# khajash/gym_puzzles

Hardware: AMD Instinct MI355X
Metric: env-steps/sec (whole node) at N envs/GPU (higher is better)
Workload: dtype f32 (engine) + f64 (env arithmetic)

## Files before the change

### gym_puzzles_amd/build.py

```python
from __future__ import annotations

import os
import re
import subprocess
import sys
from concurrent.futures import ThreadPoolExecutor

HERE = os.path.dirname(os.path.abspath(__file__))
CSRC = os.path.join(HERE, "csrc")
OUT = os.path.join(HERE, "libmrp.so")
with open(os.path.join(CSRC, "mrp_config.h")) as _f:
    N_ENVS = len(re.findall(r"^\s*X\(\d+,", _f.read(), re.M))
SOURCES = ([(f, f + ".o", None) for f in ("mrp_kernels.hip", "mrp_tables.cpp", "mrp_norm.hip")]
           + [("mrp_unit.hip", f"mrp_env{e}.o", e) for e in range(N_ENVS)])
HEADERS = ("mrp_math.h", "mrp_config.h", "mrp_world.h", "mrp_env.h", "mrp_tables.h", "mrp_ops.h", "mrp_lane.h", "mrp_render.h")


def deps(csrc: str = CSRC) -> list[str]:
    return [os.path.join(csrc, f) for f in sorted({s for s, _, _ in SOURCES}) + list(HEADERS)] + [
        os.path.join(HERE, "..", "include", "mrp.h"), os.path.abspath(__file__)]


_MAX_ILP = ["-mllvm", "-amdgpu-sched-strategy=max-ilp"]
_ILP_LOOPS = ["-DMRP_SOLVE_NOINLINE_LANES"] + _MAX_ILP
_LANES_PAIRS = ["-DMRP_LANES_PAIRS=1"]
_GRANULES = ["-DMRP_CONTACT_GRANULES=1"]
_ITER_ILP = ["-mllvm", "-amdgpu-sched-strategy=iterative-ilp"]
_BFREE = ["-DMRP_VEL_BFREE=1", "-DMRP_VEL_PICK2=1", "-DMRP_VEL_VTCROSS=1"]
_FRESH = ["-DMRP_FRESH_REGS=1"]
_BFREE_LANES = ["-DMRP_VEL_BFREE=1", "-DMRP_VEL_BFREE_LANES=1"]
_W4 = ["-DMRP_STEP_WAVES_PER_EU=4"]
UNIT_FLAGS = {0: _LANES_PAIRS + _ITER_ILP + _FRESH + _BFREE_LANES + _W4, 1: _MAX_ILP,
              2: _GRANULES + _MAX_ILP + _BFREE, 4: _ILP_LOOPS + _BFREE,
              5: _LANES_PAIRS + _ITER_ILP + _FRESH + _BFREE_LANES + _W4}
FLAGS = ["--offload-arch=gfx950", "-O3", "-std=c++17", "-ffp-contract=off", "-fno-fast-math",
         "-fno-gpu-flush-denormals-to-zero", "-fhip-fp32-correctly-rounded-divide-sqrt", "-fno-strict-aliasing",
         "-fno-slp-vectorize", "-fPIC", "-Wno-pass-failed"]


def hipcc() -> str:
    for c in (os.environ.get("HIPCC"), "/opt/rocm/bin/hipcc", "hipcc"):
        if c and (os.path.exists(c) or c == "hipcc"):
            return c
    return "hipcc"


def up_to_date() -> bool:
    if not os.path.exists(OUT):
        return False
    t = os.path.getmtime(OUT)
    return all(os.path.getmtime(d) <= t for d in deps() if os.path.exists(d))


def build(force: bool = False, verbose: bool = False, out: str = OUT, defines=(), jobs: int | None = None,
          only_envs=None, csrc: str = CSRC) -> str:
    if not force and out == OUT and up_to_date():
        return out
    objdir = os.path.join(HERE, "build", os.path.basename(out) + ".obj")
    os.makedirs(objdir, exist_ok=True)
    dflags = [f"-D{d}" for d in defines]
    srcs = [os.path.join(csrc, s) for s, _, _ in SOURCES]
    objs = [os.path.join(objdir, o) for _, o, _ in SOURCES]
    todo = list(range(len(SOURCES)))
    dep_files = deps(csrc)
    if only_envs is not None:
        assert out != OUT, "only_envs builds a variant library, never the default one"
        base = os.path.join(HERE, "build", os.path.basename(OUT) + ".obj")
        todo = [i for i, (_, _, e) in enumerate(SOURCES) if e is None or e in only_envs]
        newest_dep = max(os.path.getmtime(d) for d in dep_files if os.path.exists(d) and d.endswith((".h", ".hip", ".cpp")))
        for i, (_, o, _) in enumerate(SOURCES):
            if i not in todo:
                objs[i] = os.path.join(base, o)
                if not os.path.exists(objs[i]):
                    raise FileNotFoundError(f"{objs[i]}: build the default library first")
                if os.path.getmtime(objs[i]) < newest_dep and not os.environ.get("MRP_ALLOW_STALE_UNITS"):
                    raise RuntimeError(f"{objs[i]} is older than a source or header it depends on: rebuild the default "
                                       "library (python -m gym_puzzles_amd.build) before a variant")

    extra = os.environ.get("MRP_EXTRA_FLAGS", "").split() if out != OUT else []

    headers = [d for d in dep_files if d.endswith(".h")]
    newest_header = max(os.path.getmtime(d) for d in headers if os.path.exists(d))

    def compile_one(i: int) -> None:
        env = SOURCES[i][2]
        unit = [] if env is None else (UNIT_FLAGS.get(env, []) if not extra else []) + [f"-DMRP_ENV={env}"]
        cmd = [hipcc()] + FLAGS + unit + extra + dflags + ["-c", srcs[i], "-o", objs[i]]
        stamp = objs[i] + ".cmd"
        line = " ".join(cmd)
        if not force and os.path.exists(objs[i]) and os.path.exists(stamp):
            t = os.path.getmtime(objs[i])
            with open(stamp) as f:
                same = f.read() == line
            if same and t >= os.path.getmtime(srcs[i]) and t >= newest_header:
                return
        if verbose:
            print(line, flush=True)
        subprocess.run(cmd, check=True)
        with open(stamp, "w") as f:
            f.write(line)

    jobs = jobs or max(1, min(len(SOURCES), os.cpu_count() or 1, int(os.environ.get("MAX_JOBS", "16"))))
    order = sorted(todo, key=lambda i: SOURCES[i][2] is None)
    with ThreadPoolExecutor(jobs) as ex:
        list(ex.map(compile_one, order))
    cmd = [hipcc()] + FLAGS + ["-shared"] + objs + ["-o", out + ".tmp"]
    if verbose:
        print(" ".join(cmd), flush=True)
    subprocess.run(cmd, check=True)
    os.replace(out + ".tmp", out)
    return out


if __name__ == "__main__":
    if "--stamps" in sys.argv:
        print(build(verbose=True, out=os.path.join(HERE, "libmrp_stamps.so"), defines=("MRP_STAMPS",)))
    elif "--progress" in sys.argv:
        print(build(verbose=True, out=os.path.join(HERE, "libmrp_progress.so"), defines=("MRP_PROGRESS",)))
    elif "--variant" in sys.argv:
        i = sys.argv.index("--variant")
        args = sys.argv[i + 2:]
        envs = [int(a) for a in args if not a.startswith("-D")]
        defs = [a[2:] for a in args if a.startswith("-D")]
        print(build(verbose=True, out=os.path.abspath(sys.argv[i + 1]), defines=defs, only_envs=envs))
    else:
        print(build(force="--force" in sys.argv, verbose=True))
```

### gym_puzzles_amd/csrc/mrp_math.h

```cpp
#pragma once
#include <hip/hip_runtime.h>
#include <stdint.h>

#define MRP_HD __host__ __device__ __forceinline__

namespace mrp {

struct V2 { float x, y; };
struct Rot { float s, c; };
struct Xf { V2 p; Rot q; };

MRP_HD V2 v2(float x, float y) { V2 r; r.x = x; r.y = y; return r; }
MRP_HD V2 vadd(V2 a, V2 b) { return v2(a.x + b.x, a.y + b.y); }
MRP_HD V2 vsub(V2 a, V2 b) { return v2(a.x - b.x, a.y - b.y); }
MRP_HD V2 vmul(float s, V2 a) { return v2(s * a.x, s * a.y); }
MRP_HD V2 vneg(V2 a) { return v2(-a.x, -a.y); }
MRP_HD float vdot(V2 a, V2 b) { return a.x * b.x + a.y * b.y; }
MRP_HD float vcross(V2 a, V2 b) { return a.x * b.y - a.y * b.x; }
MRP_HD V2 vcross_vs(V2 a, float s) { return v2(s * a.y, -s * a.x); }
MRP_HD V2 vcross_sv(float s, V2 a) { return v2(-s * a.y, s * a.x); }
MRP_HD float vlensq(V2 a) { return a.x * a.x + a.y * a.y; }
MRP_HD float vlen(V2 a) { return sqrtf(a.x * a.x + a.y * a.y); }
MRP_HD float vnormalize(V2& a) {
    float length = sqrtf(a.x * a.x + a.y * a.y);
// ... 34 lines not shown
constexpr double SC_HPI_INV = 0x1.45F306DC9C883p+23, SC_HPI = 0x1.921FB54442D18p0;
constexpr double SC_C0 = 0x1p0, SC_C1 = -0x1.ffffffd0c621cp-2, SC_C2 = 0x1.55553e1068f19p-5,
                 SC_C3 = -0x1.6c087e89a359dp-10, SC_C4 = 0x1.99343027bf8c3p-16;
constexpr double SC_S1 = -0x1.555545995a603p-3, SC_S2 = 0x1.1107605230bc4p-7, SC_S3 = -0x1.994eb3774cf24p-13;

MRP_HD double sc_sign(int n) { return ((n + 1) & 2) ? -1.0 : 1.0; }

MRP_HD uint32_t f2u(float f) { union { float f; uint32_t u; } x; x.f = f; return x.u; }
MRP_HD float u2f(uint32_t u) { union { float f; uint32_t u; } x; x.u = u; return x.f; }
MRP_HD uint32_t abstop12(float x) { return (f2u(x) >> 20) & 0x7ff; }

MRP_HD float sincos_poly(double x, double x2, bool neg, int n) {
    if ((n & 1) == 0) {
        double x3 = x * x2;
        double s1 = fma(x2, SC_S3, SC_S2);
        double x7 = x3 * x2;
        double s = fma(x3, SC_S1, x);
        return (float)fma(x7, s1, s);
    } else {
        double x4 = x2 * x2;
        double c2 = fma(x2, SC_C4, SC_C3);
        double c1 = fma(x2, SC_C1, SC_C0);
        double x6 = x4 * x2;
        double c = fma(x4, SC_C2, c1);
        float r = (float)fma(x6, c2, c);
        return neg ? -r : r;
    }
}

MRP_HD double reduce_fast(double x, int* np) {
    double r = x * SC_HPI_INV;
    int n = ((int32_t)r + 0x800000) >> 24;
    *np = n;
    return fma(-(double)n, SC_HPI, x);
}

MRP_HD double reduce_large(uint32_t xi, int* np) {
    const uint32_t inv_pio4[24] = {0xa2, 0xa2f9, 0xa2f983, 0xa2f9836e, 0xf9836e4e, 0x836e4e44, 0x6e4e4415, 0x4e441529,
        0x441529fc, 0x1529fc27, 0x29fc2757, 0xfc2757d1, 0x2757d1f5, 0x57d1f534, 0xd1f534dd, 0xf534ddc0,
        0x34ddc0db, 0xddc0db62, 0xc0db6295, 0xdb629599, 0x6295993c, 0x95993c43, 0x993c4390, 0x3c439041};
    const uint32_t* arr = &inv_pio4[(xi >> 26) & 15];
    int shift = (xi >> 23) & 7;
    uint64_t n, res0, res1, res2;
    xi = (xi & 0xffffff) | 0x800000;
    xi <<= shift;
    res0 = xi * arr[0];
    res1 = (uint64_t)xi * arr[4];
    res2 = (uint64_t)xi * arr[8];
    res0 = (res2 >> 32) | (res0 << 32);
    res0 += res1;
    n = (res0 + (1ULL << 61)) >> 62;
    res0 -= n << 62;
    double x = (double)(int64_t)res0;
    *np = (int)n;
    return x * 0x1.921FB54442D18p-62;
}

MRP_HD float g_sinf(float y) {
    double x = y, s; int n;
    if (abstop12(y) < abstop12(0x1.921FB6p-1f)) {
        s = x * x;
        if (abstop12(y) < abstop12(0x1p-12f)) return y;
        return sincos_poly(x, s, false, 0);
    } else if (abstop12(y) < abstop12(120.0f)) {
        x = reduce_fast(x, &n);
        s = sc_sign(n);
        return sincos_poly(x * s, x * x, (n & 2) != 0, n);
    } else if (abstop12(y) < abstop12(__builtin_inff())) {
        uint32_t xi = f2u(y); int sign = xi >> 31;
        x = reduce_large(xi, &n);
        s = sc_sign(n + sign);
        return sincos_poly(x * s, x * x, ((n + sign) & 2) != 0, n);
    }
    return (y - y) / (y - y);
}

MRP_HD float g_cosf(float y) {
    double x = y, s; int n;
    if (abstop12(y) < abstop12(0x1.921FB6p-1f)) {
        double x2 = x * x;
        if (abstop12(y) < abstop12(0x1p-12f)) return 1.0f;
        return sincos_poly(x, x2, false, 1);
    } else if (abstop12(y) < abstop12(120.0f)) {
        x = reduce_fast(x, &n);
        s = sc_sign(n);
        return sincos_poly(x * s, x * x, (n & 2) != 0, n ^ 1);
    } else if (abstop12(y) < abstop12(__builtin_inff())) {
        uint32_t xi = f2u(y); int sign = xi >> 31;
        x = reduce_large(xi, &n);
        s = sc_sign(n + sign);
        return sincos_poly(x * s, x * x, ((n + sign) & 2) != 0, n ^ 1);
    }
    return (y - y) / (y - y);
}

MRP_HD Rot rot_fast(float y) {
    const double x = y;
    const double r = x * SC_HPI_INV;
    const int n = ((int32_t)r + 0x800000) >> 24;
    const double xr = fma(-(double)n, SC_HPI, x);
    const double xs = ((n + 1) & 2) ? -xr : xr;
    const double x2 = xr * xr;
    const double x3 = xs * x2;
    const double s1 = fma(x2, SC_S3, SC_S2);
    const double x7 = x3 * x2;
    const double ss = fma(x3, SC_S1, xs);
    const float ps = (float)fma(x7, s1, ss);
    const double x4 = x2 * x2;
    const double c2 = fma(x2, SC_C4, SC_C3);
    const double c1 = fma(x2, SC_C1, SC_C0);
    const double x6 = x4 * x2;
    const double cc = fma(x4, SC_C2, c1);
    const float pc0 = (float)fma(x6, c2, cc);
    const float pc = (n & 2) ? -pc0 : pc0;
    const bool odd = (n & 1) != 0;
    const bool tiny = abstop12(y) < abstop12(0x1p-12f);
    Rot q;
    q.s = tiny ? y : (odd ? pc : ps);
    q.c = tiny ? 1.0f : (odd ? ps : pc);
    return q;
}

MRP_HD Rot rot_slow(float y) {
    Rot q;
    double x = y;
    int n;
    const uint32_t t = abstop12(y);
    if (t < abstop12(0x1.921FB6p-1f)) {
        if (t < abstop12(0x1p-12f)) { q.s = y; q.c = 1.0f; return q; }
        const double x2 = x * x;
        q.s = sincos_poly(x, x2, false, 0);
        q.c = sincos_poly(x, x2, false, 1);
    } else if (t < abstop12(120.0f)) {
        x = reduce_fast(x, &n);
        const double s = sc_sign(n);
        q.s = sincos_poly(x * s, x * x, (n & 2) != 0, n);
        q.c = sincos_poly(x * s, x * x, (n & 2) != 0, n ^ 1);
    } else if (t < abstop12(__builtin_inff())) {
        const uint32_t xi = f2u(y);
        const int sign = xi >> 31;
        x = reduce_large(xi, &n);
        const double s = sc_sign(n + sign);
        q.s = sincos_poly(x * s, x * x, ((n + sign) & 2) != 0, n);
        q.c = sincos_poly(x * s, x * x, ((n + sign) & 2) != 0, n ^ 1);
    } else {
        q.s = (y - y) / (y - y);
        q.c = q.s;
    }
    return q;
}

MRP_HD Rot rot(float y) {
#if defined(__HIP_DEVICE_COMPILE__)
    Rot q = rot_fast(y);
    const bool big = !(abstop12(y) < abstop12(120.0f));
    if (__builtin_expect(__builtin_amdgcn_ballot_w64(big) != 0, 0)) {
        if (big) q = rot_slow(y);
    }
    return q;
#else
    if (abstop12(y) < abstop12(120.0f)) return rot_fast(y);
    return rot_slow(y);
#endif
}

MRP_HD Rot rot_z(float y) {
#if defined(__HIP_DEVICE_COMPILE__)
    if (__builtin_amdgcn_ballot_w64(y != 0.0f) == 0) { Rot q; q.s = y; q.c = 1.0f; return q; }
#endif
    return rot(y);
}

MRP_HD uint64_t splitmix64(uint64_t x) {
    x += 0x9E3779B97F4A7C15ULL;
    x = (x ^ (x >> 30)) * 0xBF58476D1CE4E5B9ULL;
    x = (x ^ (x >> 27)) * 0x94D049BB133111EBULL;
    return x ^ (x >> 31);
}
MRP_HD double rng_u01(uint64_t seed, uint64_t lane, uint64_t stream, uint64_t counter) {
    uint64_t h = splitmix64(seed ^ splitmix64(lane ^ splitmix64(stream ^ splitmix64(counter))));
    return (double)(h >> 11) * 0x1.0p-53;
}

}
```

### gym_puzzles_amd/csrc/mrp_world.h

```cpp
#pragma once
#include <type_traits>

#include "mrp_config.h"

namespace mrp {

constexpr int NULLN = -1;

#define MRP_SOLVE_FN __device__ __forceinline__
#ifdef MRP_SOLVE_NOINLINE_LANES
#define MRP_LANES_FN __device__ __attribute__((noinline))
#else
#define MRP_LANES_FN MRP_SOLVE_FN
#endif
#ifndef MRP_LANES_PAIRS
#define MRP_LANES_PAIRS 0
#endif
#ifndef MRP_VEL_PICK2
#define MRP_VEL_PICK2 0
#endif
#ifndef MRP_VEL_VTCROSS
#define MRP_VEL_VTCROSS 0
#endif
#ifndef MRP_VEL_BFREE
#define MRP_VEL_BFREE 0
#endif
#ifndef MRP_VEL_BFREE_LANES
#define MRP_VEL_BFREE_LANES 0
#endif
#ifndef MRP_FRESH_REGS
#define MRP_FRESH_REGS 0
#endif
#if MRP_VEL_VTCROSS
#define MRP_VT(dv, n, t) pcross(dv, n)
#define MRP_PT(l, n, t) ([](const P2 q_) { return p2(q_.x, -q_.y); }(pbc(l) * (n).yx))
#else
#define MRP_VT(dv, n, t) pdot(dv, t)
#define MRP_PT(l, n, t) (pbc(l) * (t))
#endif

extern "C" __device__ int mrp_writelane(int val, int lane, int old) __asm("llvm.amdgcn.writelane.i32");

#ifdef MRP_STAMPS
static __device__ unsigned long long g_stamps[16];
static __device__ unsigned long long g_pmax[16];
static __device__ unsigned long long g_stepmax[256];
static __device__ unsigned long long g_rt[2];
constexpr int MRP_TRACE_W = 40;
static __device__ uint32_t g_trace[16384][MRP_TRACE_W];
#define MRP_NOW() __builtin_amdgcn_s_memtime()
#define MRP_SUB(k, t0) do { if (tid == 0) sh.trace[k] += (uint32_t)(__builtin_amdgcn_s_memtime() - (t0)); } while (0)
#define MRP_TRACE(k, v) do { if (tid == 0) sh.trace[k] += (v); } while (0)
#define MRP_STAMP(k)                                                                        \
    do {                                                                                    \
        if (tid == 0) {                                                                     \
            unsigned long long _t = __builtin_amdgcn_s_memtime();                           \
            sh.trace[k] += (uint32_t)(_t - sh.stamp_t);                                     \
            sh.stamp_t = _t;                                                                \
        }                                                                                   \
    } while (0)
#else
#define MRP_STAMP(k) MRP_PROG(0x100u * ((k) + 1))
#define MRP_TRACE(k, v) do {} while (0)
#define MRP_NOW() 0ull
#define MRP_SUB(k, t0) do { (void)(t0); } while (0)
#endif
#ifdef MRP_PROGRESS
static __device__ uint32_t* g_progress;
#define MRP_PROG(k)                                                                                          \
    do {                                                                                                     \
        if (threadIdx.x == 0 && g_progress)                                                                  \
            __hip_atomic_store(g_progress + blockIdx.x, (uint32_t)(k), __ATOMIC_RELAXED, __HIP_MEMORY_SCOPE_SYSTEM); \
    } while (0)
#else
#define MRP_PROG(k) do {} while (0)
#endif
constexpr int MRP_FAULT_TREE_UP = 1, MRP_FAULT_TREE_DOWN = 2, MRP_FAULT_TREE_REMOVE = 3, MRP_FAULT_CONTACT_LIST = 4,
              MRP_FAULT_ISLANDS = 5, MRP_FAULT_TOI_PASSES = 6, MRP_FAULT_PAIR_DECODE = 7, MRP_FAULT_DFS = 8;
constexpr int MRP_FAULT_TREE_POOL = 9, MRP_FAULT_CONTACT_POOL = 10, MRP_FAULT_MOVE_BUFFER = 11, MRP_FAULT_ISLAND_POOL = 12;
constexpr float LINEAR_SLOP = 0.005f;
constexpr float AABB_EXT = 0.1f;
constexpr float AABB_MUL = 2.0f;
constexpr float MAX_TRANSLATION = 2.0f;
constexpr float MAX_TRANSLATION_SQ = MAX_TRANSLATION * MAX_TRANSLATION;
constexpr float B2_PI = 3.14159265359f;
constexpr float MAX_ROTATION = 0.5f * B2_PI;
constexpr float MAX_ROTATION_SQ = MAX_ROTATION * MAX_ROTATION;
constexpr float BAUMGARTE = 0.2f;
constexpr float TOI_BAUMGARTE = 0.75f;
constexpr float VELOCITY_THRESHOLD = 1.0f;
constexpr float MAX_LINEAR_CORRECTION = 0.2f;
constexpr int MAX_SUBSTEPS = 8;
constexpr int MAX_TOI_CONTACTS = 32;
constexpr float FLT_EPS = 1.1920928955078125e-7f;
constexpr float FLT_MAXV = 3.40282346638528859811704183484516925e+38f;

constexpr int CF_ISLAND = 1, CF_TOUCHING = 2, CF_ENABLED = 4, CF_TOI = 32;
constexpr int MT_FACEA = 1, MT_FACEB = 2;

template <int ENV> struct alignas(16) LaneState {
    using D = Dims<ENV>;
    static constexpr int ND = D::NA + D::NB;
    static constexpr int C = D::CMAX;
    static constexpr int TN = tree_n<ENV>();
    static constexpr int MOVE_N = move_n<ENV>();
    using PMask = typename std::conditional<(TN <= 32), uint32_t, uint64_t>::type;
    static_assert(D::NF < MOVE_N, "move buffer smaller than the proxy count");
    static_assert(D::NA + D::NB + 4 <= MAXBODY && D::NF <= MAXF, "env tables too small for this env id");
    float xpx[ND], xpy[ND], xs[ND], xc[ND];
    float c0x[ND], c0y[ND], cx[ND], cy[ND], a0[ND], a[ND], alpha0[ND];
    float vx[ND], vy[ND], w[ND];
    float fx[ND], fy[ND], tq[ND];
    int proxy[D::NF];
    float tlx[TN], tly[TN], thx[TN], thy[TN];
    int tpar[TN], tc1[TN], tc2[TN], th[TN], tud[TN];
    int root, freeList, nodeCount, moveCount;
    int moveBuf[MOVE_N];
    int cHead, cFree, cCount, cHW;
    static constexpr int NCA = 24;
    int cnext[C], cprev[C], cfa[C], cfb[C], cflags[C], ctoiCount[C];
    float ctoi[C], cfric[C];
    int mpc[C], mtype[C];
    float mlnx[C], mlny[C], mlpx[C], mlpy[C];
    float mpx[2][C], mpy[2][C], mni[2][C], mti[2][C];
    uint32_t mid[2][C];
    float inv_dt0;
    int newFixture, haveBodies, episode;
    uint32_t stepCounter;
    int elapsed, blks_in_place, prev_blks_in_place;
    int goal_contact[D::NA];
    int wall_contact;
    int fault;
    double agent_dist[D::NA];
    double block_distance[D::NB];
    double goal[D::NB][3];
    long long toiEvents, posIters;
    long long touching;
    long long nonfinite;
};

template <int ENV> constexpr int lane_words() { return (int)(sizeof(LaneState<ENV>) / 4); }

struct TOIOut { int state; float t; };

struct ClipV { V2 v; uint32_t id; };
struct VC {
    float rAx[2], rAy[2], rBx[2], rBy[2], ni[2], ti[2], nmass[2], tmass[2], vbias[2];
    float nx, ny, nm0, nm1, nm3, k0, k1, k3;
    float mA, mB, iA, iB, friction;
    int iaI, ibI, pointCount, slot;
};
struct PC {
    float lpx[2], lpy[2], lnx, lny, lpx0, lpy0;
    float lcAx, lcAy, lcBx, lcBy, rA, rB;
    int type, pointCount;
};
template <int NBODY, int C> struct IslT {
    int bodies[NBODY];
    int contacts[C];
    float pcx[NBODY], pcy[NBODY], pa[NBODY], vvx[NBODY], vvy[NBODY], vw[NBODY];
    int nb, nc;
    int index[NBODY];
};
struct SweepV { float lcx, lcy, c0x, c0y, cx, cy, a0, a, alpha0; };
struct DProxy { const V2* v; int count; float radius; };
struct SVert { V2 wA, wB, w; float a; int iA, iB; };
struct Simplex { SVert v0, v1, v2; int count; };
struct SCache { float metric; int count; int iA0, iA1, iA2, iB0, iB1, iB2; };
struct SepFn { int type; V2 lp, axis; };

template <int ENV> struct LdsTables {
    static constexpr int NF = Dims<ENV>::NF, NBODY = Dims<ENV>::NA + Dims<ENV>::NB + 4;
    ShapeDef shape[NF];
    int fix_body[NF];
    float fix_friction[NF], fix_restitution[NF];
    float invMass[NBODY], invI[NBODY], lcx[NBODY], lcy[NBODY], linDamp[NBODY], angDamp[NBODY];
    int body_fix0[NBODY], body_nfix[NBODY];
    float wall_px[4], wall_py[4];
};

template <int ENV> struct Shared {
    using D = Dims<ENV>;
    using LS = LaneState<ENV>;
    static constexpr int ND = LS::ND, NBODY = ND + 4, C = D::CMAX;
// ... 1185 lines not shown
        return sweeps;
    }
    template <bool XA0, bool XA1, int P0, int P1>
    MRP_SOLVE_FN int sweep_two(Isl& is, VC* vcs, int iters, bool early_exit, int x, int y, int z) {
        CC c0 = load_cc(vcs[0]), c1 = load_cc(vcs[1]);
        P2 vX = p2(is.vvx[x], is.vvy[x]), vY = p2(is.vvx[y], is.vvy[y]), vZ = p2(is.vvx[z], is.vvy[z]);
        float wX = is.vw[x], wY = is.vw[y], wZ = is.vw[z];
        const int sweeps = sweep_pairs<17>(iters, early_exit, [&] {
            if (XA0) cc_update<P0>(c0, vX, wX, vY, wY); else cc_update<P0>(c0, vY, wY, vX, wX);
            if (XA1) cc_update<P1>(c1, vX, wX, vZ, wZ); else cc_update<P1>(c1, vZ, wZ, vX, wX);
        }, [&](float (&v)[17]) {
            v[0] = vX.x; v[1] = vX.y; v[2] = wX; v[3] = vY.x; v[4] = vY.y; v[5] = wY; v[6] = vZ.x; v[7] = vZ.y; v[8] = wZ;
            v[9] = c0.ni.x; v[10] = c0.ni.y; v[11] = c0.ti.x; v[12] = c0.ti.y; v[13] = c1.ni.x; v[14] = c1.ni.y; v[15] = c1.ti.x; v[16] = c1.ti.y;
        });
        if (tid == 0) {
            is.vvx[x] = vX.x; is.vvy[x] = vX.y; is.vw[x] = wX;
            is.vvx[y] = vY.x; is.vvy[y] = vY.y; is.vw[y] = wY;
            is.vvx[z] = vZ.x; is.vvy[z] = vZ.y; is.vw[z] = wZ;
            store_cc(vcs[0], c0); store_cc(vcs[1], c1);
        }
        return sweeps;
    }
    template <bool SAME, int P0, int P1>
    MRP_SOLVE_FN int sweep_same(Isl& is, VC* vcs, int iters, bool early_exit, int p, int q) {
        CC c0 = load_cc(vcs[0]), c1 = load_cc(vcs[1]);
        P2 vP = p2(is.vvx[p], is.vvy[p]), vQ = p2(is.vvx[q], is.vvy[q]);
        float wP = is.vw[p], wQ = is.vw[q];
        const int sweeps = sweep_pairs<14>(iters, early_exit, [&] {
            cc_update<P0>(c0, vP, wP, vQ, wQ);
            if (SAME) cc_update<P1>(c1, vP, wP, vQ, wQ); else cc_update<P1>(c1, vQ, wQ, vP, wP);
        }, [&](float (&v)[14]) {
            v[0] = vP.x; v[1] = vP.y; v[2] = wP; v[3] = vQ.x; v[4] = vQ.y; v[5] = wQ;
            v[6] = c0.ni.x; v[7] = c0.ni.y; v[8] = c0.ti.x; v[9] = c0.ti.y; v[10] = c1.ni.x; v[11] = c1.ni.y; v[12] = c1.ti.x; v[13] = c1.ti.y;
        });
        if (tid == 0) {
            is.vvx[p] = vP.x; is.vvy[p] = vP.y; is.vw[p] = wP;
            is.vvx[q] = vQ.x; is.vvy[q] = vQ.y; is.vw[q] = wQ;
            store_cc(vcs[0], c0); store_cc(vcs[1], c1);
        }
        return sweeps;
    }
    template <int P0, int P1>
    __device__ __forceinline__ int solver_velocity_two_p(Isl& is, VC* vcs, int iters, bool early_exit) {
        const int a0 = vcs[0].iaI, b0 = vcs[0].ibI, a1 = vcs[1].iaI, b1 = vcs[1].ibI;
        if (a0 == a1 && b0 == b1) return sweep_same<true, P0, P1>(is, vcs, iters, early_exit, a0, b0);
        if (a0 == b1 && b0 == a1) return sweep_same<false, P0, P1>(is, vcs, iters, early_exit, a0, b0);
        if (a0 == a1) return sweep_two<true, true, P0, P1>(is, vcs, iters, early_exit, a0, b0, b1);
        if (a0 == b1) return sweep_two<true, false, P0, P1>(is, vcs, iters, early_exit, a0, b0, a1);
        if (b0 == a1) return sweep_two<false, true, P0, P1>(is, vcs, iters, early_exit, b0, a0, b1);
        if (b0 == b1) return sweep_two<false, false, P0, P1>(is, vcs, iters, early_exit, b0, a0, a1);
        return -1;
    }
    __device__ __forceinline__ int solver_velocity_two(Isl& is, VC* vcs, int iters, bool early_exit = true) {
        const int p0 = __builtin_amdgcn_readfirstlane(vcs[0].pointCount), p1 = __builtin_amdgcn_readfirstlane(vcs[1].pointCount);
        if (p0 == 2) return p1 == 2 ? solver_velocity_two_p<2, 2>(is, vcs, iters, early_exit)
                                    : solver_velocity_two_p<2, 1>(is, vcs, iters, early_exit);
        return p1 == 2 ? solver_velocity_two_p<1, 2>(is, vcs, iters, early_exit)
                       : solver_velocity_two_p<1, 1>(is, vcs, iters, early_exit);
    }

    __device__ __forceinline__ static P2 rot_cs(float angle) { const Rot q = rot(angle); return p2(q.c, q.s); }
    __device__ __forceinline__ static P2 prot(P2 q, P2 v) { return q * pbc(v.x) + pperp(q) * pbc(v.y); }
    struct RotMemo {
        uint32_t k0 = 0u, k1 = 0u;
        P2 q0 = {1.0f, 0.0f}, q1 = {1.0f, 0.0f};
        bool next1 = false;
        __device__ __forceinline__ P2 get(float angle) {
            const uint32_t b = __float_as_uint(angle);
            if (b == 0u) return p2(1.0f, 0.0f);
            if (b == k0) { next1 = true; return q0; }
            if (b == k1) { next1 = false; return q1; }
            const P2 q = rot_cs(angle);
            if (next1) { k1 = b; q1 = q; } else { k0 = b; q0 = q; }
            next1 = !next1;
            return q;
        }
    };
    struct UniMemo {
        uint32_t k0 = 0u, k1 = 0u;
        P2 q0 = {1.0f, 0.0f}, q1 = {1.0f, 0.0f};
        bool next1 = false;
        __device__ __forceinline__ P2 get(float angle) {
            const uint32_t b = __float_as_uint(angle);
            if (uni(b == 0u)) return p2(1.0f, 0.0f);
            if (uni(b == k0)) { next1 = true; return q0; }
            if (uni(b == k1)) { next1 = false; return q1; }
            const P2 q = rot_cs(angle);
            if (next1) { k1 = b; q1 = q; } else { k0 = b; q0 = q; }
            next1 = !next1;
            return q;
        }
    };
    struct PCC {
        P2 lcA, lcB, ln, lp0, q0, q1;
        P2 mA, mB;
        float radA, radB, iA, iB;
        int pcount, type;
    };
    __device__ __forceinline__ static PCC load_pcc(const VC& vc, const PC& pc, bool toi, int toiA, int toiB) {
        PCC o;
        o.lcA = p2(pc.lcAx, pc.lcAy); o.lcB = p2(pc.lcBx, pc.lcBy);
        o.ln = p2(pc.lnx, pc.lny); o.lp0 = p2(pc.lpx0, pc.lpy0);
        o.q0 = p2(pc.lpx[0], pc.lpy[0]); o.q1 = p2(pc.lpx[1], pc.lpy[1]);
        o.radA = pc.rA; o.radB = pc.rB;
        float mA = vc.mA, iA = vc.iA, mB = vc.mB, iB = vc.iB;
        if (toi) {
            if (!(vc.iaI == toiA || vc.iaI == toiB)) { mA = 0.0f; iA = 0.0f; }
            if (!(vc.ibI == toiA || vc.ibI == toiB)) { mB = 0.0f; iB = 0.0f; }
        }
        o.mA = pbc(mA); o.iA = iA; o.mB = pbc(mB); o.iB = iB;
        o.pcount = pc.pointCount;
        o.type = pc.type;
        return o;
    }
    template <class Rots, class OnSep>
    __device__ __forceinline__ static void pos_update(const PCC& c, int pcount, int type, float baum, Rots&& rots,
                                                      OnSep onSep, P2& cA, float& aA, P2& cB, float& aB) {
        const P2 mA = c.mA, mB = c.mB;
        const float iA = c.iA, iB = c.iB;
        for (int j = 0; j < 2; ++j) {
            if (j == pcount) break;
            P2 qA, qB;
            rots(aA, aB, qA, qB);
            const P2 pA = cA - prot(qA, c.lcA), pB = cB - prot(qB, c.lcB);
            const P2 lp = j == 0 ? c.q0 : c.q1;
            P2 normal, point; float sep;
            if (type == MT_FACEA) {
                normal = prot(qA, c.ln);
                const P2 planePoint = prot(qA, c.lp0) + pA;
                const P2 clipPoint = prot(qB, lp) + pB;
                sep = pdot(clipPoint - planePoint, normal) - c.radA - c.radB;
                point = clipPoint;
            } else {
                normal = prot(qB, c.ln);
                const P2 planePoint = prot(qB, c.lp0) + pB;
                const P2 clipPoint = prot(qA, lp) + pA;
                sep = pdot(clipPoint - planePoint, normal) - c.radA - c.radB;
                point = clipPoint;
                normal = -normal;
            }
            const P2 rA = point - cA, rB = point - cB;
            onSep(sep);
            const float Cc = fclamp(baum * (sep + LINEAR_SLOP), -MAX_LINEAR_CORRECTION, 0.0f);
            const float rnA = pcross(rA, normal), rnB = pcross(rB, normal);
            const float K = mA.x + mB.x + iA * rnA * rnA + iB * rnB * rnB;
            const float impulse = K > 0.0f ? -Cc / K : 0.0f;
            const P2 Pv = pbc(impulse) * normal;
            cA = cA - mA * Pv;
            aA -= iA * pcross(rA, Pv);
            cB = cB + mB * Pv;
            aB += iB * pcross(rB, Pv);
        }
    }
    template <class Rots>
    __device__ __forceinline__ static void pcc_update(const PCC& c, P2& cA, float& aA, P2& cB, float& aB, float& minSep,
                                                      float baum, Rots&& rots) {
        pos_update(c, c.pcount, c.type, baum, rots, [&minSep](float sep) { minSep = fmin_(minSep, sep); }, cA, aA, cB, aB);
    }
    template <int NC, bool SAMEB, bool XA0, bool XA1>
    MRP_SOLVE_FN int pos_sweep(Isl& is, const VC* vcs, const PC* pcs, bool toi, int toiA, int toiB, int iters,
                                             int p, int q, int z) {
        PCC c0 = load_pcc(vcs[0], pcs[0], toi, toiA, toiB);
        PCC c1 = load_pcc(vcs[NC - 1], pcs[NC - 1], toi, toiA, toiB);
        c0.pcount = __builtin_amdgcn_readfirstlane(c0.pcount); c0.type = __builtin_amdgcn_readfirstlane(c0.type);
        c1.pcount = __builtin_amdgcn_readfirstlane(c1.pcount); c1.type = __builtin_amdgcn_readfirstlane(c1.type);
        P2 cP = p2(is.pcx[p], is.pcy[p]), cQ = p2(is.pcx[q], is.pcy[q]), cZ = p2(is.pcx[z], is.pcy[z]);
        float aP = is.pa[p], aQ = is.pa[q], aZ = is.pa[z];
        const float baum = toi ? TOI_BAUMGARTE : BAUMGARTE;
        const float exitSep = toi ? -1.5f * LINEAR_SLOP : -3.0f * LINEAR_SLOP;
        auto pass = [&](auto&& with) {
            float minSep = 0.0f;
            if (NC == 1 || SAMEB) {
                if (XA0) with(0, [&](auto&& r) { pcc_update(c0, cP, aP, cQ, aQ, minSep, baum, r); });
                else with(0, [&](auto&& r) { pcc_update(c0, cQ, aQ, cP, aP, minSep, baum, r); });
                if (NC == 2) {
                    if (XA1) with(1, [&](auto&& r) { pcc_update(c1, cP, aP, cQ, aQ, minSep, baum, r); });
                    else with(1, [&](auto&& r) { pcc_update(c1, cQ, aQ, cP, aP, minSep, baum, r); });
                }
            } else {
                if (XA0) with(0, [&](auto&& r) { pcc_update(c0, cP, aP, cQ, aQ, minSep, baum, r); });
                else with(0, [&](auto&& r) { pcc_update(c0, cQ, aQ, cP, aP, minSep, baum, r); });
                if (XA1) with(1, [&](auto&& r) { pcc_update(c1, cP, aP, cZ, aZ, minSep, baum, r); });
                else with(1, [&](auto&& r) { pcc_update(c1, cZ, aZ, cP, aP, minSep, baum, r); });
            }
            return minSep;
        };
        int it = 0;
        UniMemo memo;
        while (it < iters) {
            ++it;
            const float minSep = pass([&memo](int, auto&& upd) {
                upd([&memo](float a, float b, P2& qa, P2& qb) { qa = memo.get(a); qb = memo.get(b); });
            });
            if (uni(minSep >= exitSep)) break;
        }
        if (tid == 0) {
            is.pcx[p] = cP.x; is.pcy[p] = cP.y; is.pa[p] = aP;
            is.pcx[q] = cQ.x; is.pcy[q] = cQ.y; is.pa[q] = aQ;
            if (NC == 2 && !SAMEB) { is.pcx[z] = cZ.x; is.pcy[z] = cZ.y; is.pa[z] = aZ; }
        }
        return it;
    }
    __device__ __forceinline__ int solver_position_small(Isl& is, const VC* vcs, const PC* pcs, bool toi, int toiA, int toiB,
                                                         int iters) {
        const int nc = __builtin_amdgcn_readfirstlane(is.nc);
        const int a0 = vcs[0].iaI, b0 = vcs[0].ibI;
        if (nc == 1) return pos_sweep<1, true, true, true>(is, vcs, pcs, toi, toiA, toiB, iters, a0, b0, b0);
        if (nc != 2) return -1;
        const int a1 = vcs[1].iaI, b1 = vcs[1].ibI;
        if (a0 == a1 && b0 == b1) return pos_sweep<2, true, true, true>(is, vcs, pcs, toi, toiA, toiB, iters, a0, b0, b0);
        if (a0 == b1 && b0 == a1) return pos_sweep<2, true, true, false>(is, vcs, pcs, toi, toiA, toiB, iters, a0, b0, b0);
        if (a0 == a1) return pos_sweep<2, false, true, true>(is, vcs, pcs, toi, toiA, toiB, iters, a0, b0, b1);
        if (a0 == b1) return pos_sweep<2, false, true, false>(is, vcs, pcs, toi, toiA, toiB, iters, a0, b0, a1);
        if (b0 == a1) return pos_sweep<2, false, false, true>(is, vcs, pcs, toi, toiA, toiB, iters, b0, a0, b1);
        if (b0 == b1) return pos_sweep<2, false, false, false>(is, vcs, pcs, toi, toiA, toiB, iters, b0, a0, a1);
        return -1;
    }

    template <class Contact>
    __device__ __forceinline__ int lanes_pass_loop(int iters, float exitSep, Contact&& contact) {
        int it = 0;
        RotMemo memo;
        while (it < iters) {
            ++it;
            const float minSep = contact([&memo](int i, auto&& upd) {
                upd([&memo, i](float a, float b, P2& qa, P2& qb) { qa = memo.get(rdl(a, i)); qb = memo.get(rdl(b, i)); });
            });
            if (minSep >= exitSep) break;
        }
        return it;
    }
    template <int NC>
    MRP_LANES_FN int lanes_passes(Isl& is, const VC* vcs, const PC* pcs, bool toi, int toiA, int toiB, int iters) {
        const int me = tid < NC ? tid : 0;
        const PCC my = load_pcc(vcs[me], pcs[me], toi, toiA, toiB);
        const int cia = vcs[me].iaI, cib = vcs[me].ibI;
        const int bk = tid < is.nb ? tid : 0;
        float bx = is.pcx[bk], by = is.pcy[bk], ba = is.pa[bk];
        const float baum = toi ? TOI_BAUMGARTE : BAUMGARTE;
        const float exitSep = toi ? -1.5f * LINEAR_SLOP : -3.0f * LINEAR_SLOP;
        int ia[NC], ib[NC], pc[NC], ty[NC];
#pragma unroll
        for (int i = 0; i < NC; ++i) { ia[i] = rdli(cia, i); ib[i] = rdli(cib, i); pc[i] = rdli(my.pcount, i); ty[i] = rdli(my.type, i); }
        const int it = lanes_pass_loop(iters, exitSep, [&](auto&& with) {
            float minSep = 0.0f;
#pragma unroll
            for (int i = 0; i < NC; ++i) {
                P2 cA = p2(rdl(bx, ia[i]), rdl(by, ia[i])); float aA = rdl(ba, ia[i]);
                P2 cB = p2(rdl(bx, ib[i]), rdl(by, ib[i])); float aB = rdl(ba, ib[i]);
                with(i, [&](auto&& rots) {
                    pos_update(my, pc[i], ty[i], baum, rots, [&minSep, i](float sep) { minSep = fmin_(minSep, rdl(sep, i)); },
                               cA, aA, cB, aB);
                });
                bx = wrl(bx, rdl(cA.x, i), ia[i]); by = wrl(by, rdl(cA.y, i), ia[i]); ba = wrl(ba, rdl(aA, i), ia[i]);
                bx = wrl(bx, rdl(cB.x, i), ib[i]); by = wrl(by, rdl(cB.y, i), ib[i]); ba = wrl(ba, rdl(aB, i), ib[i]);
            }
            return minSep;
        });
        if (tid < is.nb) { is.pcx[tid] = bx; is.pcy[tid] = by; is.pa[tid] = ba; }
        return it;
    }
    __device__ __forceinline__ int solver_position_lanes(Isl& is, const VC* vcs, const PC* pcs, bool toi, int toiA, int toiB, int iters) {
        if constexpr (NB == 1) {
            const int n = __builtin_amdgcn_readfirstlane(is.nc);
            if (n == 3) return lanes_passes<3>(is, vcs, pcs, toi, toiA, toiB, iters);
            if (n == 4) return lanes_passes<4>(is, vcs, pcs, toi, toiA, toiB, iters);
        }
        const int nc = is.nc;
        const int me = tid < nc ? tid : 0;
        const PCC my = load_pcc(vcs[me], pcs[me], toi, toiA, toiB);
        const int cia = vcs[me].iaI, cib = vcs[me].ibI;
        const int bk = tid < is.nb ? tid : 0;
        float bx = is.pcx[bk], by = is.pcy[bk], ba = is.pa[bk];
        const float baum = toi ? TOI_BAUMGARTE : BAUMGARTE;
        const float exitSep = toi ? -1.5f * LINEAR_SLOP : -3.0f * LINEAR_SLOP;
        const int ncu = __builtin_amdgcn_readfirstlane(nc);
        const int it = lanes_pass_loop(iters, exitSep, [&](auto&& with) {
            float minSep = 0.0f;
            for (int i = 0; i < ncu; ++i) {
                const int ia = rdli(cia, i), ib = rdli(cib, i), pcount = rdli(my.pcount, i), type = rdli(my.type, i);
                P2 cA = p2(rdl(bx, ia), rdl(by, ia)); float aA = rdl(ba, ia);
                P2 cB = p2(rdl(bx, ib), rdl(by, ib)); float aB = rdl(ba, ib);
                with(i, [&](auto&& rots) {
                    pos_update(my, pcount, type, baum, rots, [&minSep, i](float sep) { minSep = fmin_(minSep, rdl(sep, i)); },
                               cA, aA, cB, aB);
                });
                bx = wrl(bx, rdl(cA.x, i), ia); by = wrl(by, rdl(cA.y, i), ia); ba = wrl(ba, rdl(aA, i), ia);
                bx = wrl(bx, rdl(cB.x, i), ib); by = wrl(by, rdl(cB.y, i), ib); ba = wrl(ba, rdl(aB, i), ib);
            }
            return minSep;
        });
        if (tid < is.nb) { is.pcx[tid] = bx; is.pcy[tid] = by; is.pa[tid] = ba; }
        return it;
    }

    __device__ __forceinline__ void integrate_positions(Isl& is, float h) {
        for (int i = 0; i < is.nb; ++i) {
            V2 c = v2(is.pcx[i], is.pcy[i]); float a = is.pa[i];
            V2 v = v2(is.vvx[i], is.vvy[i]); float w = is.vw[i];
            V2 translation = vmul(h, v);
            if (vdot(translation, translation) > MAX_TRANSLATION_SQ) {
                float ratio = MAX_TRANSLATION / vlen(translation);
                v.x *= ratio; v.y *= ratio;
            }
            float rotation = h * w;
            if (rotation * rotation > MAX_ROTATION_SQ) {
                float ratio = MAX_ROTATION / fabsf(rotation);
                w *= ratio;
            }
            c = vadd(c, vmul(h, v));
            a += h * w;
            is.pcx[i] = c.x; is.pcy[i] = c.y; is.pa[i] = a;
            is.vvx[i] = v.x; is.vvy[i] = v.y; is.vw[i] = w;
        }
    }
    __device__ __forceinline__ void island_add_body(Isl& is, int b) { is.index[b] = is.nb; is.bodies[is.nb++] = b; }

    __device__ __forceinline__ void island_pre(Isl& is, float h, float dtRatio, VC* vcs, PC* pcs) {
        for (int i = 0; i < is.nb; ++i) {
            int b = is.bodies[i];
            if (is_dyn(b)) {
                V2 c = v2(S.cx[b], S.cy[b]); float a = S.a[b];
                V2 v = v2(S.vx[b], S.vy[b]); float w = S.w[b];
                S.c0x[b] = S.cx[b]; S.c0y[b] = S.cy[b]; S.a0[b] = S.a[b];
                V2 g = v2(1.0f * 0.0f, 1.0f * 0.0f);
                V2 acc = vadd(g, vmul(L.invMass[b], v2(S.fx[b], S.fy[b])));
                v = vadd(v, vmul(h, acc));
                w += h * L.invI[b] * S.tq[b];
                { float s = 1.0f / (1.0f + h * L.linDamp[b]); v.x *= s; v.y *= s; }
                w *= 1.0f / (1.0f + h * L.angDamp[b]);
                is.pcx[i] = c.x; is.pcy[i] = c.y; is.pa[i] = a; is.vvx[i] = v.x; is.vvy[i] = v.y; is.vw[i] = w;
            } else {
                V2 c = center(b);
                is.pcx[i] = c.x; is.pcy[i] = c.y; is.pa[i] = 0.0f; is.vvx[i] = 0.0f; is.vvy[i] = 0.0f; is.vw[i] = 0.0f;
            }
        }
        MRP_TRACE(12, is.nc);
        if (is.nc > 0) {
            solver_init(is, vcs, pcs, true, dtRatio);
            solver_init_velocity(is, vcs, pcs);
            solver_warm_start(is, vcs);
        }
    }
    __device__ __forceinline__ void island_mid(Isl& is, float h, VC* vcs) {
        if (is.nc > 0) solver_store(is, vcs);
        integrate_positions(is, h);
    }
    __device__ __forceinline__ void island_position(Isl& is, VC* vcs, PC* pcs, int nc) {
        if (nc > 0 && nc <= 64) {
            int n = solver_position_small(is, vcs, pcs, false, -1, -1, 60);
            if (n < 0) n = solver_position_lanes(is, vcs, pcs, false, -1, -1, 60);
            if (tid == 0) S.posIters += n;
        } else if (tid == 0) {
            if (nc > 0) {
                for (int it = 0; it < 60; ++it) {
                    ++S.posIters;
                    if (solver_position(is, vcs, pcs, false, -1, -1)) break;
                }
            } else {
                ++S.posIters;
            }
        }
    }
    __device__ __forceinline__ void island_post(Isl& is) {
        for (int i = 0; i < is.nb; ++i) {
            int b = is.bodies[i];
            if (!is_dyn(b)) continue;
            S.cx[b] = is.pcx[i]; S.cy[b] = is.pcy[i]; S.a[b] = is.pa[i];
            S.vx[b] = is.vvx[i]; S.vy[b] = is.vvy[i]; S.w[b] = is.vw[i];
            sync_transform(b);
        }
    }

    static constexpr int NLW = (C + 63) / 64;
    __device__ __forceinline__ void solve_coop(float h, float dtRatio) {
        static_assert(BLOCK == 64, "a workgroup is one wave: that alone orders the wave's reads after thread 0's writes");
        Isl& is = sh.isl;
        uint32_t bflag = 0;
        int seed = ND - 1;
        const int nl = sh.ccount;
        uint64_t joined[NLW];
#pragma unroll
        for (int w = 0; w < NLW; ++w) joined[w] = 0ull;
        for (int nisl = 0;; ++nisl) {
            MRP_PROG(0x3000u + nisl);
            refresh_tid();
            if (nisl > NBODY + 1) { if (tid == 0) S.fault = MRP_FAULT_ISLANDS; break; }
            while (seed >= 0 && (bflag & (1u << seed))) --seed;
            if (seed < 0) break;
            const unsigned long long td = MRP_NOW();
            int nb = 0, ncs = 0, sc = 0, stk = 0;
            uint32_t statics = 0u;
            stk = seed; sc = 1; bflag |= 1u << seed;
            int lslot[NLW], lA[NLW], lB[NLW];
            bool lok[NLW];
#pragma unroll
            for (int w = 0; w < NLW; ++w) {
                const int k = tid + 64 * w;
                const bool live = k < nl && sh.cover[k];
                const int c = live ? sh.clist[k] : 0;
                lslot[w] = c;
                lA[w] = live ? (int)L.fix_body[S.cfa[c]] : -1;
                lB[w] = live ? (int)L.fix_body[S.cfb[c]] : -1;
                const int f = live ? S.cflags[c] : 0;
                lok[w] = live && (f & CF_ENABLED) != 0 && (f & CF_TOUCHING) != 0;
            }
            for (int g = 0; sc > 0; ++g) {
                if (g > 2 * NBODY) { if (tid == 0) S.fault = MRP_FAULT_DFS; break; }
                const int b = __builtin_amdgcn_readlane(stk, sc - 1);
                --sc;
                if (tid == 0) { is.index[b] = nb; is.bodies[nb] = b; }
                ++nb;
                if (!is_dyn(b)) { statics |= 1u << b; continue; }
#pragma unroll
                for (int w = 0; w < NLW; ++w) {
                    uint64_t m = __builtin_amdgcn_ballot_w64(lok[w] && (lA[w] == b || lB[w] == b)) & ~joined[w];
                    for (int q = 0; m != 0ull && q < 64; ++q) {
                        const int l = (int)__builtin_ctzll(m);
                        m &= m - 1ull;
                        if (ncs >= C || sc >= NBODY) { if (tid == 0) S.fault = MRP_FAULT_ISLAND_POOL; continue; }
                        const int c = __builtin_amdgcn_readlane(lslot[w], l);
                        const int other = __builtin_amdgcn_readlane(lA[w] == b ? lB[w] : lA[w], l);
                        if (tid == 0) is.contacts[ncs] = c;
                        ++ncs;
                        joined[w] |= 1ull << l;
                        if (bflag & (1u << other)) continue;
                        stk = mrp_writelane(other, sc, stk);
                        ++sc;
                        bflag |= 1u << other;
                    }
                }
            }
            if (tid == 0) {
                is.nb = nb; is.nc = ncs;
                MRP_SUB(32, td);
                const unsigned long long tp = MRP_NOW();
                island_pre(is, h, dtRatio, sh.u.sol.vcs, sh.u.sol.pcs);
                MRP_SUB(18, tp);
#ifdef MRP_STAMPS
                if ((uint32_t)is.nc > sh.trace[19]) sh.trace[19] = (uint32_t)is.nc;
#endif
            }
            __syncthreads();
            const int nc = __builtin_amdgcn_readfirstlane(is.nc);
            const unsigned long long tv = MRP_NOW();
            const int lvl = nc >= 6 ? 3 : (nc >= 4 ? 2 : (nc >= 2 ? 1 : 0));
            if (nc > 0 && nc <= 64) {
// ... 587 lines not shown
```

Baseline: 24.94 million.

## Specialize lane position solver for static bodies with pre-rotated contact geometry

Adds an MRP_FIXED_SIDES mode, enabled for env unit 1. For contacts where a body has zero inverse inertia, its local contact geometry is pre-rotated into world frame once, so each position-solver iteration skips that body's rotation lookup and angular update. A wave-wide validity check falls back to the generic path when bounds are violated. The rot() path also computes rot_fast on a sanitized input for large angles. The cost is more code, extra branching per contact, and possible rounding differences because rotation is applied once up front rather than every pass.

Result: no change. 24.87 million (-0.3%).

```diff
diff --git a/gym_puzzles_amd/build.py b/gym_puzzles_amd/build.py
--- a/gym_puzzles_amd/build.py
+++ b/gym_puzzles_amd/build.py
@@ -30,7 +30,8 @@
 _FRESH = ["-DMRP_FRESH_REGS=1"]
 _BFREE_LANES = ["-DMRP_VEL_BFREE=1", "-DMRP_VEL_BFREE_LANES=1"]
 _W4 = ["-DMRP_STEP_WAVES_PER_EU=4"]
-UNIT_FLAGS = {0: _LANES_PAIRS + _ITER_ILP + _FRESH + _BFREE_LANES + _W4, 1: _MAX_ILP,
+_FIXED = ["-DMRP_FIXED_SIDES=1"]
+UNIT_FLAGS = {0: _LANES_PAIRS + _ITER_ILP + _FRESH + _BFREE_LANES + _W4, 1: _MAX_ILP + _FIXED,
               2: _GRANULES + _MAX_ILP + _BFREE, 4: _ILP_LOOPS + _BFREE,
               5: _LANES_PAIRS + _ITER_ILP + _FRESH + _BFREE_LANES + _W4}
 FLAGS = ["--offload-arch=gfx950", "-O3", "-std=c++17", "-ffp-contract=off", "-fno-fast-math",
diff --git a/gym_puzzles_amd/csrc/mrp_math.h b/gym_puzzles_amd/csrc/mrp_math.h
--- a/gym_puzzles_amd/csrc/mrp_math.h
+++ b/gym_puzzles_amd/csrc/mrp_math.h
@@ -210,8 +210,13 @@
 
 MRP_HD Rot rot(float y) {
 #if defined(__HIP_DEVICE_COMPILE__)
+#if defined(MRP_FIXED_SIDES) && MRP_FIXED_SIDES
+    const bool big = !(abstop12(y) < abstop12(120.0f));
+    Rot q = rot_fast(big ? 0.0f : y);
+#else
     Rot q = rot_fast(y);
     const bool big = !(abstop12(y) < abstop12(120.0f));
+#endif
     if (__builtin_expect(__builtin_amdgcn_ballot_w64(big) != 0, 0)) {
         if (big) q = rot_slow(y);
     }
diff --git a/gym_puzzles_amd/csrc/mrp_world.h b/gym_puzzles_amd/csrc/mrp_world.h
--- a/gym_puzzles_amd/csrc/mrp_world.h
+++ b/gym_puzzles_amd/csrc/mrp_world.h
@@ -30,6 +30,9 @@
 #endif
 #ifndef MRP_FRESH_REGS
 #define MRP_FRESH_REGS 0
+#endif
+#ifndef MRP_FIXED_SIDES
+#define MRP_FIXED_SIDES 0
 #endif
 #if MRP_VEL_VTCROSS
 #define MRP_VT(dv, n, t) pcross(dv, n)
@@ -1521,6 +1524,78 @@
             aB += iB * pcross(rB, Pv);
         }
     }
+#if MRP_FIXED_SIDES
+    static constexpr float FS_POS = 0x1p39f, FS_MLO = 0x1p-20f, FS_MHI = 0x1p20f;
+    __device__ __forceinline__ static bool fs_mass_ok(float m) { return __float_as_uint(m) == 0u || (m >= FS_MLO && m <= FS_MHI); }
+    __device__ __forceinline__ static bool fs_inertia_ok(float i) { return __float_as_uint(i) == 0u || (i > 0.0f && i <= FS_MHI); }
+    __device__ __forceinline__ static bool fs_p2_ok(P2 v, float bound) { return fabsf(v.x) <= bound && fabsf(v.y) <= bound; }
+    __device__ __forceinline__ static bool fs_contact_ok(const PCC& c) {
+        const bool pts = fs_p2_ok(c.lcA, FS_POS) && fs_p2_ok(c.lcB, FS_POS) && fs_p2_ok(c.lp0, FS_POS) &&
+                         fs_p2_ok(c.q0, FS_POS) && fs_p2_ok(c.q1, FS_POS) && fs_p2_ok(c.ln, 2.0f);
+        const bool mass = fs_mass_ok(c.mA.x) && fs_mass_ok(c.mB.x) && fs_inertia_ok(c.iA) && fs_inertia_ok(c.iB);
+        const bool both0 = __float_as_uint(c.iA) == 0u && __float_as_uint(c.iB) == 0u;
+        return pts && mass && (c.mA.x + c.mB.x > 0.0f || both0);
+    }
+    __device__ __forceinline__ static bool fs_body_ok(float x, float y, float a) {
+        return fabsf(x) <= FS_POS && fabsf(y) <= FS_POS && fabsf(a) <= FS_POS;
+    }
+    __device__ __forceinline__ static void fixed_sides(PCC& c, bool island_ok, float aA, float aB, bool& fA, bool& fB) {
+        fA = island_ok && __float_as_uint(c.iA) == 0u && __float_as_uint(aA) != 0x80000000u;
+        fB = island_ok && __float_as_uint(c.iB) == 0u && __float_as_uint(aB) != 0x80000000u;
+        const Rot rA = rot_z(fA ? aA : 0.0f), rB = rot_z(fB ? aB : 0.0f);
+        const P2 qA = p2(rA.c, rA.s), qB = p2(rB.c, rB.s);
+        const bool faceA = c.type == MT_FACEA;
+        const bool refFixed = faceA ? fA : fB, incFixed = faceA ? fB : fA;
+        const P2 qRef = faceA ? qA : qB, qInc = faceA ? qB : qA;
+        const P2 lcA = prot(qA, c.lcA), lcB = prot(qB, c.lcB);
+        const P2 ln = prot(qRef, c.ln), lp0 = prot(qRef, c.lp0), q0 = prot(qInc, c.q0), q1 = prot(qInc, c.q1);
+        c.lcA = fA ? lcA : c.lcA; c.lcB = fB ? lcB : c.lcB;
+        c.ln = refFixed ? ln : c.ln; c.lp0 = refFixed ? lp0 : c.lp0;
+        c.q0 = incFixed ? q0 : c.q0; c.q1 = incFixed ? q1 : c.q1;
+    }
+    template <bool FA, bool FB, class One, class OnSep>
+    __device__ __forceinline__ static void pos_update_fixed(const PCC& c, int pcount, int type, float baum, One&& one,
+                                                            OnSep onSep, P2& cA, float& aA, P2& cB, float& aB) {
+        static_assert(FA || FB, "the generic form is pos_update");
+        const P2 mA = c.mA, mB = c.mB;
+        const float iA = c.iA, iB = c.iB;
+        for (int j = 0; j < 2; ++j) {
+            if (j == pcount) break;
+            P2 qA = {}, qB = {};
+            if (!FA) qA = one(aA);
+            if (!FB) qB = one(aB);
+            const P2 pA = cA - (FA ? c.lcA : prot(qA, c.lcA)), pB = cB - (FB ? c.lcB : prot(qB, c.lcB));
+            const P2 lp = j == 0 ? c.q0 : c.q1;
+            P2 normal, point; float sep;
+            if (type == MT_FACEA) {
+                normal = FA ? c.ln : prot(qA, c.ln);
+                const P2 planePoint = (FA ? c.lp0 : prot(qA, c.lp0)) + pA;
+                const P2 clipPoint = (FB ? lp : prot(qB, lp)) + pB;
+                sep = pdot(clipPoint - planePoint, normal) - c.radA - c.radB;
+                point = clipPoint;
+            } else {
+                normal = FB ? c.ln : prot(qB, c.ln);
+                const P2 planePoint = (FB ? c.lp0 : prot(qB, c.lp0)) + pB;
+                const P2 clipPoint = (FA ? lp : prot(qA, lp)) + pA;
+                sep = pdot(clipPoint - planePoint, normal) - c.radA - c.radB;
+                point = clipPoint;
+                normal = -normal;
+            }
+            onSep(sep);
+            const float Cc = fclamp(baum * (sep + LINEAR_SLOP), -MAX_LINEAR_CORRECTION, 0.0f);
+            float K = mA.x + mB.x;
+            P2 rA = {}, rB = {};
+            if (!FA) { rA = point - cA; const float rnA = pcross(rA, normal); K = K + iA * rnA * rnA; }
+            if (!FB) { rB = point - cB; const float rnB = pcross(rB, normal); K = K + iB * rnB * rnB; }
+            const float impulse = K > 0.0f ? -Cc / K : 0.0f;
+            const P2 Pv = pbc(impulse) * normal;
+            cA = cA - mA * Pv;
+            if (!FA) aA -= iA * pcross(rA, Pv);
+            cB = cB + mB * Pv;
+            if (!FB) aB += iB * pcross(rB, Pv);
+        }
+    }
+#endif
     template <class Rots>
     __device__ __forceinline__ static void pcc_update(const PCC& c, P2& cA, float& aA, P2& cB, float& aB, float& minSep,
                                                       float baum, Rots&& rots) {
@@ -1586,6 +1661,123 @@
         return -1;
     }
 
+#if MRP_FIXED_SIDES
+    struct LaneRots {
+        RotMemo& memo;
+        int i;
+        __device__ __forceinline__ void operator()(float a, float b, P2& qa, P2& qb) const { qa = memo.get(rdl(a, i)); qb = memo.get(rdl(b, i)); }
+        __device__ __forceinline__ P2 one(float a) const { return memo.get(rdl(a, i)); }
+    };
+    template <class Contact>
+    __device__ __forceinline__ int lanes_pass_loop(int iters, float exitSep, Contact&& contact) {
+        int it = 0;
+        RotMemo memo;
+        while (it < iters) {
+            ++it;
+            const float minSep = contact([&memo](int i, auto&& upd) { upd(LaneRots{memo, i}); });
+            if (minSep >= exitSep) break;
+        }
+        return it;
+    }
+    template <class Rots, class OnSep>
+    __device__ __forceinline__ static void lanes_pos_update(const PCC& c, bool fa, bool fb, int pcount, int type, float baum,
+                                                            Rots&& rots, OnSep onSep, P2& cA, float& aA, P2& cB, float& aB) {
+#if MRP_FIXED_SIDES
+        auto one = [&rots](float a) { return rots.one(a); };
+        if (fa && fb) return pos_update_fixed<true, true>(c, pcount, type, baum, one, onSep, cA, aA, cB, aB);
+        if (fa) return pos_update_fixed<true, false>(c, pcount, type, baum, one, onSep, cA, aA, cB, aB);
+        if (fb) return pos_update_fixed<false, true>(c, pcount, type, baum, one, onSep, cA, aA, cB, aB);
+#endif
+        pos_update(c, pcount, type, baum, rots, onSep, cA, aA, cB, aB);
+    }
+    __device__ __forceinline__ static void lanes_fixed_sides(PCC& my, float bx, float by, float ba, float aA, float aB,
+                                                             bool& fA, bool& fB) {
+        const bool ok = __builtin_amdgcn_ballot_w64(!(fs_contact_ok(my) && fs_body_ok(bx, by, ba))) == 0;
+        fixed_sides(my, ok, aA, aB, fA, fB);
+    }
+    template <int NC>
+    MRP_LANES_FN int lanes_passes(Isl& is, const VC* vcs, const PC* pcs, bool toi, int toiA, int toiB, int iters) {
+        const int me = tid < NC ? tid : 0;
+        PCC my = load_pcc(vcs[me], pcs[me], toi, toiA, toiB);
+        const int cia = vcs[me].iaI, cib = vcs[me].ibI;
+        const int bk = tid < is.nb ? tid : 0;
+        float bx = is.pcx[bk], by = is.pcy[bk], ba = is.pa[bk];
+        const float baum = toi ? TOI_BAUMGARTE : BAUMGARTE;
+        const float exitSep = toi ? -1.5f * LINEAR_SLOP : -3.0f * LINEAR_SLOP;
+        int ia[NC], ib[NC], pc[NC], ty[NC];
+        bool fa[NC], fb[NC];
+#pragma unroll
+        for (int i = 0; i < NC; ++i) { ia[i] = rdli(cia, i); ib[i] = rdli(cib, i); pc[i] = rdli(my.pcount, i); ty[i] = rdli(my.type, i); fa[i] = fb[i] = false; }
+#if MRP_FIXED_SIDES
+        {
+            bool fA, fB;
+            lanes_fixed_sides(my, bx, by, ba, is.pa[cia], is.pa[cib], fA, fB);
+            const uint64_t mA = __builtin_amdgcn_ballot_w64(fA), mB = __builtin_amdgcn_ballot_w64(fB);
+#pragma unroll
+            for (int i = 0; i < NC; ++i) { fa[i] = (mA >> i) & 1ull; fb[i] = (mB >> i) & 1ull; }
+        }
+#endif
+        const int it = lanes_pass_loop(iters, exitSep, [&](auto&& with) {
+            float minSep = 0.0f;
+#pragma unroll
+            for (int i = 0; i < NC; ++i) {
+                P2 cA = p2(rdl(bx, ia[i]), rdl(by, ia[i])); float aA = rdl(ba, ia[i]);
+                P2 cB = p2(rdl(bx, ib[i]), rdl(by, ib[i])); float aB = rdl(ba, ib[i]);
+                with(i, [&](auto&& rots) {
+                    lanes_pos_update(my, fa[i], fb[i], pc[i], ty[i], baum, rots,
+                                     [&minSep, i](float sep) { minSep = fmin_(minSep, rdl(sep, i)); }, cA, aA, cB, aB);
+                });
+                bx = wrl(bx, rdl(cA.x, i), ia[i]); by = wrl(by, rdl(cA.y, i), ia[i]); if (!fa[i]) ba = wrl(ba, rdl(aA, i), ia[i]);
+                bx = wrl(bx, rdl(cB.x, i), ib[i]); by = wrl(by, rdl(cB.y, i), ib[i]); if (!fb[i]) ba = wrl(ba, rdl(aB, i), ib[i]);
+            }
+            return minSep;
+        });
+        if (tid < is.nb) { is.pcx[tid] = bx; is.pcy[tid] = by; is.pa[tid] = ba; }
+        return it;
+    }
+    __device__ __forceinline__ int solver_position_lanes(Isl& is, const VC* vcs, const PC* pcs, bool toi, int toiA, int toiB, int iters) {
+        if constexpr (NB == 1) {
+            const int n = __builtin_amdgcn_readfirstlane(is.nc);
+            if (n == 3) return lanes_passes<3>(is, vcs, pcs, toi, toiA, toiB, iters);
+            if (n == 4) return lanes_passes<4>(is, vcs, pcs, toi, toiA, toiB, iters);
+        }
+        const int nc = is.nc;
+        const int me = tid < nc ? tid : 0;
+        PCC my = load_pcc(vcs[me], pcs[me], toi, toiA, toiB);
+        const int cia = vcs[me].iaI, cib = vcs[me].ibI;
+        const int bk = tid < is.nb ? tid : 0;
+        float bx = is.pcx[bk], by = is.pcy[bk], ba = is.pa[bk];
+        uint64_t fmA = 0ull, fmB = 0ull;
+#if MRP_FIXED_SIDES
+        {
+            bool fA, fB;
+            lanes_fixed_sides(my, bx, by, ba, is.pa[cia], is.pa[cib], fA, fB);
+            fmA = __builtin_amdgcn_ballot_w64(fA); fmB = __builtin_amdgcn_ballot_w64(fB);
+        }
+#endif
+        const float baum = toi ? TOI_BAUMGARTE : BAUMGARTE;
+        const float exitSep = toi ? -1.5f * LINEAR_SLOP : -3.0f * LINEAR_SLOP;
+        const int ncu = __builtin_amdgcn_readfirstlane(nc);
+        const int it = lanes_pass_loop(iters, exitSep, [&](auto&& with) {
+            float minSep = 0.0f;
+            for (int i = 0; i < ncu; ++i) {
+                const int ia = rdli(cia, i), ib = rdli(cib, i), pcount = rdli(my.pcount, i), type = rdli(my.type, i);
+                P2 cA = p2(rdl(bx, ia), rdl(by, ia)); float aA = rdl(ba, ia);
+                P2 cB = p2(rdl(bx, ib), rdl(by, ib)); float aB = rdl(ba, ib);
+                const bool fa = (fmA >> i) & 1ull, fb = (fmB >> i) & 1ull;
+                with(i, [&](auto&& rots) {
+                    lanes_pos_update(my, fa, fb, pcount, type, baum, rots,
+                                     [&minSep, i](float sep) { minSep = fmin_(minSep, rdl(sep, i)); }, cA, aA, cB, aB);
+                });
+                bx = wrl(bx, rdl(cA.x, i), ia); by = wrl(by, rdl(cA.y, i), ia); if (!fa) ba = wrl(ba, rdl(aA, i), ia);
+                bx = wrl(bx, rdl(cB.x, i), ib); by = wrl(by, rdl(cB.y, i), ib); if (!fb) ba = wrl(ba, rdl(aB, i), ib);
+            }
+            return minSep;
+        });
+        if (tid < is.nb) { is.pcx[tid] = bx; is.pcy[tid] = by; is.pa[tid] = ba; }
+        return it;
+    }
+#else
     template <class Contact>
     __device__ __forceinline__ int lanes_pass_loop(int iters, float exitSep, Contact&& contact) {
         int it = 0;
@@ -1662,6 +1854,7 @@
         if (tid < is.nb) { is.pcx[tid] = bx; is.pcy[tid] = by; is.pa[tid] = ba; }
         return it;
     }
+#endif
 
     __device__ __forceinline__ void integrate_positions(Isl& is, float h) {
         for (int i = 0; i < is.nb; ++i) {
```
